# z619850002/CVIDS

Hardware: AMD Instinct MI355X
Metric: depth frames/sec integrated + Mvoxel-updates/sec, 640x480 @ 1 cm, 1/2/4/8 GPU (higher is better)
Workload: dtype f32; 1 GPU; 640x480 depth+BGR colour stream (sphere_room, 1 agent), 1 cm voxels, chunk 16^3, InverseTruncator(1), carving 0.05 m, projective TSDF integration + marching cubes every 10 frames; image=640x480, chunk=16, color=True, frames_per_call=10, mesh_every=10, parallelism=1 GPU

## Files before the change

### cvids_amd/capi.py

```python
import ctypes as C
import os
import subprocess

_HERE = os.path.dirname(os.path.abspath(__file__))
_LIB = os.path.join(_HERE, os.environ.get("CHISEL_HIP_LIB", "libchisel_hip.so"))

ABI_VERSION = 3
NUM_COUNTERS = 9
COUNTER_NAMES = ["sdf", "col", "col_sat", "probe", "carved", "work_chunks", "new_chunks", "updated_chunks", "frames"]
NUM_KERNELS = 6
KERNEL_NAMES = ["pyramid", "cull", "integrate", "mesh", "resolve", "cloud"]
TRUNC_CONSTANT, TRUNC_INVERSE, TRUNC_QUADRATIC = 0, 1, 2
STATUS = {0: "OK", 1: "ERR_INVALID", 2: "ERR_HIP", 3: "ERR_POOL_FULL", 4: "ERR_NOT_FOUND", 5: "ERR_UNSUPPORTED", 6: "ERR_IO"}


class ChiselHipError(RuntimeError):
    def __init__(self, code, msg):
        super().__init__("chisel_hip: %s (%d): %s" % (STATUS.get(code, "?"), code, msg))
        self.code = code


class Config(C.Structure):
    _fields_ = [("chunk_size", C.c_int * 3), ("voxel_resolution", C.c_float), ("use_color", C.c_int),
                ("device_id", C.c_int), ("max_chunks", C.c_int64), ("n_shards", C.c_int), ("shard_rank", C.c_int),
# ... 66 lines not shown
    "chisel_hip_meshes_to_update", "chisel_hip_meshes_to_update_since", "chisel_hip_meshes_to_update_prefetch", "chisel_hip_shell_plan_device", "chisel_hip_shell_segment_bytes", "chisel_hip_export_shells_packed", "chisel_hip_import_shells_packed", "chisel_hip_update_meshes_planned", "chisel_hip_shell_plan_queue", "chisel_hip_import_shells_fixed", "chisel_hip_shell_commit", "chisel_hip_num_meshes", "chisel_hip_list_meshes", "chisel_hip_mesh_size",
    "chisel_hip_download_mesh", "chisel_hip_get_sdf", "chisel_hip_get_sdf_and_gradient", "chisel_hip_save_ply",
    "chisel_hip_save_map", "chisel_hip_load_map",
    "chisel_hip_drop_ghost_chunks", "chisel_hip_update_meshes_of", "chisel_hip_condition_depth", "chisel_hip_condition_color", "chisel_hip_publish_cloud",
    "chisel_hip_depth_filter_create", "chisel_hip_depth_filter_destroy", "chisel_hip_depth_filter_update", "chisel_hip_depth_filter_read",
    "chisel_hip_stereo_default_params", "chisel_hip_stereo_create", "chisel_hip_stereo_destroy", "chisel_hip_stereo_set_reference",
    "chisel_hip_stereo_update", "chisel_hip_stereo_output", "chisel_hip_stereo_clear", "chisel_hip_stereo_read",
    "chisel_hip_stereo_set_camera", "chisel_hip_stereo_set_reference_image", "chisel_hip_stereo_update_image",
    "chisel_hip_stereo_bind_sparse_points", "chisel_hip_stereo_output_image", "chisel_hip_stereo_homography",
    "chisel_hip_get_counters", "chisel_hip_memory_statistics", "chisel_hip_topology_epoch", "chisel_hip_candidates", "chisel_hip_cloud_candidates", "chisel_hip_mesh_cube", "chisel_hip_write_mesh_ply", "chisel_hip_shade_vertices", "chisel_hip_generate_mesh", "chisel_hip_recompute_mesh", "chisel_hip_integrate_chunk", "chisel_hip_dirty_ids_device", "chisel_hip_mesh_shell_plan",
    "chisel_hip_shell_volume", "chisel_hip_set_profiling", "chisel_hip_get_profile", "chisel_hip_get_launch_stats", "chisel_hip_pool_info", "chisel_hip_mc_tables", "chisel_hip_mesh_cube_values", "chisel_hip_interpolate_vertex", "chisel_hip_raycast", "chisel_hip_chunk_owner", "chisel_hip_frustum", "chisel_hip_frustum_from_vectors", "chisel_hip_create_group", "chisel_hip_render_view",
    "chisel_hip_query_points", "chisel_hip_cast_rays", "chisel_hip_align_terms", "chisel_hip_align_solve", "chisel_hip_align_depth",
]
SELFTEST_EXPORTS = [
    "chisel_hip_kat_truncation", "chisel_hip_kat_dist", "chisel_hip_kat_color", "chisel_hip_kat_color_fresh", "chisel_hip_kat_color_any",
    "chisel_hip_kat_reciprocal", "chisel_hip_kat_floor", "chisel_hip_kat_raycast", "chisel_hip_debug_cloud_stats",
    "chisel_hip_debug_cull_space", "chisel_hip_debug_frustum_range", "chisel_hip_debug_stereo_prep",
]


def library_path():
    return _LIB


def build_library(force=False):
    src_dir = os.path.join(_HERE, "csrc")
    if not force and os.path.exists(_LIB):
        newest = max(os.path.getmtime(os.path.join(src_dir, f)) for f in os.listdir(src_dir))
        newest = max(newest, os.path.getmtime(os.path.join(_HERE, "..", "include", "chisel_hip.h")))
        if os.path.getmtime(_LIB) >= newest:
            return _LIB
# ... 115 lines not shown
    L.chisel_hip_kat_truncation.argtypes = [C.c_int, C.c_float, f32p, C.c_int, f32p, f32p]
    L.chisel_hip_kat_dist.argtypes = [f32p, C.c_int, f32p]
    L.chisel_hip_kat_color.argtypes = [u8p, C.c_int, u8p]
    for name, types in (("chisel_hip_wait_event", [vp, vp]), ("chisel_hip_record_event", [vp, vp]),
                        ("chisel_hip_order_stream_after_map", [vp, vp]), ("chisel_hip_order_map_after_stream", [vp, vp]),
                        ("chisel_hip_query_points", [vp, vp, C.c_int64, vp, vp, vp, vp, vp, C.c_int]),
                        ("chisel_hip_cast_rays", [vp, vp, C.c_int64, C.c_float, vp, vp, vp, vp, C.c_int]),
                        ("chisel_hip_align_terms", [vp, C.POINTER(DepthFrame), C.c_float, vp, C.c_int]),
                        ("chisel_hip_align_solve", [C.POINTER(C.c_double), C.c_double, C.POINTER(C.c_double)]),
                        ("chisel_hip_align_depth", [vp, C.POINTER(DepthFrame), C.POINTER(AlignParams), C.POINTER(AlignResult)]),
                        ("chisel_hip_kat_color_fresh", [C.POINTER(C.c_uint)]),
                        ("chisel_hip_kat_color_any", [C.POINTER(C.c_uint)]),
                        ("chisel_hip_debug_cloud_stats", [vp, i64p]),
                        ("chisel_hip_kat_raycast", [f32p, C.c_int, i32p, i32p, i32p, C.c_int, i32p]),
                        ("chisel_hip_kat_reciprocal", [C.POINTER(C.c_ulonglong), C.POINTER(C.c_uint)]),
                        ("chisel_hip_kat_floor", [C.POINTER(C.c_ulonglong), C.POINTER(C.c_uint)])):
        try:
            getattr(L, name).argtypes = types
        except AttributeError:
            pass
    L.chisel_hip_frustum.argtypes = [f32p, C.c_float, C.c_float, C.c_int, C.c_int, C.c_float, C.c_float, f32p, f32p, f32p]
    L.chisel_hip_debug_frustum_range.argtypes = [f32p, C.c_float, C.c_float, C.c_float, C.c_float, C.c_int, C.c_int,
                                                 C.c_int, C.c_float, i32p, i32p, f32p, f32p]
    _lib = L
    return L


def check(rc):
    if rc != 0:
        raise ChiselHipError(rc, load_library().chisel_hip_last_error().decode(errors="replace"))
```

### cvids_amd/csrc/chisel_device.h

```cpp
#pragma once
#include <hip/hip_runtime.h>
#include <stdint.h>

namespace chisel_hip {

constexpr uint64_t KEY_EMPTY = ~0ull;
constexpr uint64_t KEY_TOMB = ~0ull - 1ull;
constexpr int ID_BIAS = 1 << 20;
constexpr int INTEGRATE_MAX_GRID = 4096;
constexpr int INTEGRATE_GRID_CAP = 1 << 19;

__host__ __device__ inline uint64_t pack_id(int x, int y, int z) {
    return (uint64_t)(uint32_t)(x + ID_BIAS) | ((uint64_t)(uint32_t)(y + ID_BIAS) << 21) |
           ((uint64_t)(uint32_t)(z + ID_BIAS) << 42);
}
__host__ __device__ inline void unpack_id(uint64_t k, int &x, int &y, int &z) {
    x = (int)(k & 0x1FFFFF) - ID_BIAS;
    y = (int)((k >> 21) & 0x1FFFFF) - ID_BIAS;
    z = (int)((k >> 42) & 0x1FFFFF) - ID_BIAS;
}
__host__ __device__ inline uint64_t chunk_hash(int x, int y, int z) {
    return ((uint64_t)(int64_t)x * 73856093ull) ^ ((uint64_t)(int64_t)y * 19349663ull) ^
           ((uint64_t)(int64_t)z * 8349279ull);
}
// ... 184 lines not shown
        double r = (double)reading;
        double v = (double)kQuadTerm * (r * r) + (double)(kLinTerm * reading) + (double)kConstTerm;
        v = v < 0 ? -v : v;
        return (float)(v * (double)param);
    }
}
__device__ inline float reciprocal_in_range(float z) {
    const float r = __builtin_amdgcn_rcpf(z);
    return __builtin_fmaf(__builtin_fmaf(-z, r, 1.0f), r, r);
}
__device__ inline int floor_to_int(float x) {
    int r;
    asm("v_cvt_flr_i32_f32 %0, %1" : "=v"(r) : "v"(x));
    return r;
}
constexpr float FASTZ_MIN = 9.094947017729282e-13f;
constexpr float FASTZ_MAX = 1099511627776.0f;
__host__ __device__ inline float constant_weight(float weight, float truncation) { return weight / (5 * truncation); }
__host__ __device__ inline void dist_integrate(float &sdf, float &w, float distUpdate, float weightUpdate) {
    float newDist = (w * sdf + weightUpdate * distUpdate) / (weightUpdate + w);
    sdf = newDist;
    w = w + weightUpdate;
}
__host__ __device__ inline uint8_t color_channel(uint8_t old, uint8_t weight, uint8_t nw, uint8_t weightUpdate) {
    const unsigned x = (unsigned)weight * (unsigned)old + (unsigned)weightUpdate * (unsigned)nw;
    const unsigned d = (unsigned)weightUpdate + (unsigned)weight;
    if (d == 0u) return 0;
    const unsigned q = x / d;
    return (uint8_t)(q > 255u ? 255u : q);
}
// ... 37 lines not shown
    return *reinterpret_cast<const unaligned_u32 *>(data + lo);
}
__device__ inline unsigned color_word(unsigned raw, unsigned shift) {
    const unsigned v = raw >> shift;
    return ((v >> 16) & 0xffu) | (v & 0xff00u) | ((v & 0xffu) << 16);
}

__device__ inline unsigned color_gather2(const uint8_t *data, unsigned idx, unsigned channels, unsigned last_word, unsigned &shift) {
    const unsigned b = __umul24(idx, channels);
    const unsigned lo = b < last_word ? b : last_word;
    shift = (b - lo) * 8u;
    return *reinterpret_cast<const unaligned_u32 *>(data + lo);
}
__device__ inline unsigned color_integrate_fresh_bgr(unsigned c, unsigned v) {
    const float wf = (float)(c >> 24);
    const float r = __builtin_amdgcn_rcpf(wf + 1.0f);
    const float hr = __builtin_fmaf(0.5f, r, -0.5f);
    const float x0 = __builtin_fmaf(wf, (float)(c & 0xffu), (float)((v >> 16) & 0xffu));
    const float x1 = __builtin_fmaf(wf, (float)((c >> 8) & 0xffu), (float)((v >> 8) & 0xffu));
    const float x2 = __builtin_fmaf(wf, (float)((c >> 16) & 0xffu), (float)(v & 0xffu));
    unsigned q = c + 0x01000000u;
    q = __builtin_amdgcn_cvt_pk_u8_f32(__builtin_fmaf(x0, r, hr), 0u, q);
    q = __builtin_amdgcn_cvt_pk_u8_f32(__builtin_fmaf(x1, r, hr), 1u, q);
    q = __builtin_amdgcn_cvt_pk_u8_f32(__builtin_fmaf(x2, r, hr), 2u, q);
    return q;
}

__host__ __device__ inline bool sdf_below_carve_threshold(float sdf) { return sdf <= 1e-5f; }

}
```

### cvids_amd/csrc/chisel_hip.hip

```cpp
#include "../../include/chisel_hip.h"
#include "../../include/chisel_hip_selftest.h"

#include <hip/hip_runtime.h>
#include <hip/hip_ext.h>
#include <dlfcn.h>

#include <algorithm>
#include <array>
#include <atomic>
#include <chrono>
#include <condition_variable>
#include <functional>
#include <mutex>
#include <thread>
#include <cmath>
#include <cstdlib>
#include <cstdio>
#include <cstring>
#include <fstream>
#include <map>
#include <string>
#include <unordered_map>
#include <set>
#include <unordered_set>
// ... 2327 lines not shown
    if (ph[15])
        fprintf(stderr, "integrate_kernel phases, us per wave: item %.2f frames %.2f deposit %.2f store+or %.2f dequeue %.2f | alive %.2f | waves %llu units/wave %.2f\n",
                ph[9] * 0.01 / ph[15], ph[10] * 0.01 / ph[15], ph[11] * 0.01 / ph[15], ph[12] * 0.01 / ph[15], ph[13] * 0.01 / ph[15],
                ph[14] * 0.01 / ph[15], (unsigned long long)ph[15], (double)out[5] * 16.0 / ph[15]);
    if (ph[15])
        fprintf(stderr, "   units %llu (%.2f per wave)  frames visited %.2f per unit, executed %.2f per unit (%.2f us each), with a band update %.2f per unit\n",
                (unsigned long long)ph[19], (double)ph[19] / ph[15], (double)ph[16] / ph[19], (double)ph[17] / ph[19], ph[17] ? ph[18] * 0.01 / ph[17] : 0.0, (double)ph[20] / ph[19]);
    if (ph[15]) {
        uint64_t u[6] = {0, 0, 0, 0, 0, 0};
        for (int b = 0; b < 64; b++)
            for (int c = 0; c < 3; c++) { u[c] += rows[(size_t)b * 16 + 13 + c]; u[3 + c] += rows[(size_t)(64 + b) * 16 + 13 + c]; }
        const double ex = (double)ph[17];
        fprintf(stderr, "   per executed wave-frame: lanes needed %.1f / 64, voxels with a record %.1f / 256, voxels in band or carve test %.1f / 256; band code run by %.2f of them with %.1f lanes, carve code by %.2f with %.1f lanes\n",
                u[0] / ex, u[1] / ex, u[2] / ex, ph[20] / ex, ph[20] ? (double)u[3] / ph[20] : 0.0, u[5] / ex, u[5] ? (double)u[4] / u[5] : 0.0);
    }
    {
        unsigned long long mp[8];
        if (hipMemcpyFromSymbol(mp, HIP_SYMBOL(g_mesh_phase), sizeof(mp)) == hipSuccess && mp[7]) {
            fprintf(stderr, "mesh_count_kernel, us per job (thread 0): lookups %.2f | corners staged %.2f | cubes classified %.2f | scan %.2f | reserve %.2f | records %.2f | jobs %llu\n",
                    mp[0] * 0.01 / mp[7], mp[1] * 0.01 / mp[7], mp[2] * 0.01 / mp[7], mp[3] * 0.01 / mp[7], mp[4] * 0.01 / mp[7], mp[5] * 0.01 / mp[7], mp[7]);
            unsigned long long z[8] = {0, 0, 0, 0, 0, 0, 0, 0};
            (void)hipMemcpyToSymbol(HIP_SYMBOL(g_mesh_phase), z, sizeof(z));
        }
        if (hipMemcpyFromSymbol(mp, HIP_SYMBOL(g_tri_phase), sizeof(mp)) == hipSuccess && mp[7]) {
            fprintf(stderr, "mesh_triangle_kernel, us per wave (lane 0): prefix + search %.2f | record, job row, position %.2f | corners, three vertices %.2f | gradient %.2f | colour %.2f | waves sampled %llu\n",
                    mp[0] * 0.01 / mp[7], mp[1] * 0.01 / mp[7], mp[2] * 0.01 / mp[7], mp[3] * 0.01 / mp[7], mp[4] * 0.01 / mp[7], mp[7]);
            unsigned long long z[8] = {0, 0, 0, 0, 0, 0, 0, 0};
            (void)hipMemcpyToSymbol(HIP_SYMBOL(g_tri_phase), z, sizeof(z));
        }
    }
// ... 300 lines not shown
```

### cvids_amd/csrc/host_selftest.h

```cpp
extern "C" {

int chisel_hip_kat_truncation(int kind, float param, const float *depths, int n, float *trunc, float *weight1) {
    DeviceBuffer<float> d_in, d_t, d_w;
    HIP_TRY(d_in.alloc(n));
    HIP_TRY(d_t.alloc(n));
    HIP_TRY(d_w.alloc(n));
    HIP_TRY(hipMemcpy(d_in.get(), depths, n * sizeof(float), hipMemcpyHostToDevice));
    hipLaunchKernelGGL(kat_truncation_kernel, dim3((n + 255) / 256), dim3(256), 0, 0, kind, param, d_in.get(), n, d_t.get(), d_w.get());
    HIP_TRY(hipMemcpy(trunc, d_t.get(), n * sizeof(float), hipMemcpyDeviceToHost));
    HIP_TRY(hipMemcpy(weight1, d_w.get(), n * sizeof(float), hipMemcpyDeviceToHost));
    return CHISEL_HIP_OK;
}
int chisel_hip_kat_dist(const float *ops, int n, float *out) {
    DeviceBuffer<float> d_in, d_out;
    HIP_TRY(d_in.alloc(n * 3));
    HIP_TRY(d_out.alloc(n * 2));
    HIP_TRY(hipMemcpy(d_in.get(), ops, n * 3 * sizeof(float), hipMemcpyHostToDevice));
    hipLaunchKernelGGL(kat_dist_kernel, dim3(1), dim3(64), 0, 0, d_in.get(), n, d_out.get());
    HIP_TRY(hipMemcpy(out, d_out.get(), n * 2 * sizeof(float), hipMemcpyDeviceToHost));
    return CHISEL_HIP_OK;
}
int chisel_hip_kat_raycast(const float *rays, int n, const int lo[3], const int hi[3], int *cells, int cap, int *count) {
    DeviceBuffer<float> d_in;
    DeviceBuffer<int> d_cells, d_count;
// ... 67 lines not shown
    HIP_TRY(hipMemcpy(example_bits, e.get(), sizeof(unsigned), hipMemcpyDeviceToHost));
    return CHISEL_HIP_OK;
}
int chisel_hip_kat_floor(unsigned long long *mismatches, unsigned *example_bits) {
    DeviceBuffer<unsigned long long> d;
    DeviceBuffer<unsigned> e;
    HIP_TRY(d.alloc(1));
    HIP_TRY(e.alloc(1));
    HIP_TRY(hipMemset(d.get(), 0, sizeof(unsigned long long)));
    HIP_TRY(hipMemset(e.get(), 0, sizeof(unsigned)));
    hipLaunchKernelGGL(kat_floor_kernel, dim3(4096), dim3(256), 0, 0, d.get(), e.get());
    HIP_TRY(hipMemcpy(mismatches, d.get(), sizeof(unsigned long long), hipMemcpyDeviceToHost));
    HIP_TRY(hipMemcpy(example_bits, e.get(), sizeof(unsigned), hipMemcpyDeviceToHost));
    return CHISEL_HIP_OK;
}
int chisel_hip_debug_cull_space(const int range_min[3], const int range_dim[3], int n_shards, int shard_rank, int shard_block, int *ids,
                                int capacity, int *count) {
    CullParams P;
    memset(&P, 0, sizeof(P));
    for (int a = 0; a < 3; a++) {
        P.range_min[a] = range_min[a];
        P.range_dim[a] = range_dim[a];
    }
    P.ip.n_shards = n_shards;
    P.ip.shard_rank = shard_rank;
    P.ip.shard_block = shard_block;
    const CullSpace space(P);
    int n = 0;
    for (int c = 0; c < space.total; c++) {
        int x, y, z;
// ... 21 lines not shown
```

### cvids_amd/csrc/kernels_integrate.h

```cpp
#pragma once
#include <type_traits>

#include "chisel_device.h"
#include "kernels_cull.h"
#include "kernels_map.h"

namespace chisel_hip {

#ifndef INTEGRATE_WAVES
#define INTEGRATE_WAVES 6
#endif
#ifndef INTEGRATE_BLOCKS_PER_CU
#define INTEGRATE_BLOCKS_PER_CU 6
#endif
#ifndef INTEGRATE_WPB
#define INTEGRATE_WPB 1
#endif
#ifndef INTEGRATE_FINE_BELOW
#define INTEGRATE_FINE_BELOW 600
#endif

#ifndef INTEGRATE_PIPE
#define INTEGRATE_PIPE 0
#endif
#ifndef OPT_INSIDE
#define OPT_INSIDE 1
#endif
#ifndef OPT_ENDZ
#define OPT_ENDZ 1
#endif
#ifndef OPT_CARVESKIP
#define OPT_CARVESKIP 1
#endif
#ifndef OPT_COLOR2
#define OPT_COLOR2 1
#endif

constexpr int QUEUE_STRIDE = 32;
constexpr int QUEUE_HEADS = 128;

template <int N, int VPL>
struct Geom {
    static_assert(VPL == 4 || VPL == 2, "voxels per lane");
    static constexpr int V = N * N * N;
    static constexpr int QX = N / VPL;
    static constexpr int QUADS = V / VPL;
    static constexpr int LAYER_QUADS = QX * N;
    static constexpr int WPC = QUADS / 64;
    static_assert(QUADS % 64 == 0, "whole waves");
    static constexpr int BX = 2 * VPL, BY = 8, BZ = 4;
    static constexpr int NBX = N / BX, NBY = N / BY, NBZ = N / BZ;
    static_assert(NBX * NBY * NBZ == WPC && NBX >= 1 && NBY >= 1 && NBZ >= 1, "bricks tile the chunk");
// ... 153 lines not shown
            units_x = n_coarse_x * G::WPC + (n_x - n_coarse_x) * GF::WPC;
        }
    }
    const int rem_chunks = mixed ? 0 : n_items - grid_waves / G::WPC;
    const IntegratorParams &ip = P.ip;
    unsigned t_sdf = 0, t_col = 0, t_colsat = 0, t_probe = 0, t_carved = 0;
    unsigned n_new = 0, n_updated = 0;
    int shard_try = 0;
#ifdef CHISEL_PHASES
    unsigned long long ph_last_start = 0, ph_max_unit = 0, ph_exec0 = 0;
    int ph_wid = 0;
    unsigned long long ph_visit = 0, ph_exec = 0, ph_exec_t = 0, ph_units = 0, ph_band = 0, ph_fr_t = 0;
    unsigned long long ph_f[5] = {0, 0, 0, 0, 0}, ph_ft = 0;
#define FSTAMP(i, dep) do { asm volatile("" ::"v"(dep)); const unsigned long long n_ = __builtin_amdgcn_s_memrealtime(); ph_f[i] += n_ - ph_ft; ph_ft = n_; } while (0)
    unsigned long long ph_need_l = 0, ph_vox = 0, ph_band_l = 0, ph_carve_w = 0, ph_carve_l = 0, ph_bandcarve_v = 0;
    unsigned long long ph[6] = {0, 0, 0, 0, 0, 0}, ph_t = __builtin_amdgcn_s_memrealtime(), ph_t0 = ph_t;
#define PHASE(i) do { const unsigned long long n_ = __builtin_amdgcn_s_memrealtime(); ph[i] += n_ - ph_t; ph_t = n_; } while (0)
#else
#define PHASE(i) do { } while (0)
#define FSTAMP(i, dep) do { } while (0)
#endif

    auto run_unit = [&](auto vpl_tag, const int it, const int wq, const int wid) {
            constexpr int VPL = decltype(vpl_tag)::value;
            using G = Geom<N, VPL>;
            using QuadF = QuadFT<VPL>;
            using QuadU = QuadUT<VPL>;
            PHASE0(1, n_items);
            const WorkItem wi = items[it];
            int cr_flags = 0;
// ... 50 lines not shown
#pragma unroll
            for (int j = 0; j < VPL; j++) {
                s4.v[j] = 99999.0f;
                w4.v[j] = 0.0f;
                c4.v[j] = 0u;
            }
            constexpr unsigned HAVE = 1u, HAVEC = 2u, DCHG = 4u, CCHG = 8u;
            unsigned st = existed ? 0u : (HAVE | HAVEC);
            const size_t slot_base = (size_t)(existed ? slot : 0) * G::V;
            const unsigned lane_off = (unsigned)((vz * N + vy) * N + vx0);
            unsigned bm = 0u, cm = 0u;
            int carve_v = 0;

            struct Proj {
                int k, flags;
                bool need;
                float pcz[VPL];
                unsigned off[VPL];
                PixelRec r[VPL];
            };
            auto project = [&](const int k) -> Proj {
                Proj pj;
                pj.k = k;
#ifdef CHISEL_PHASES
                ph_ft = __builtin_amdgcn_s_memrealtime();
                ph_fr_t = ph_ft;
                ph_visit++;
#endif
                const int flags = __builtin_amdgcn_readlane(cr_flags, k);
                pj.flags = flags;
                const FrameCam &F = P.f[k];
                const CameraParams &C = F.cam;
                const float dy = wy - C.t[1], dz = wz - C.t[2];
                const float s2 = C.R[5] * dy + C.R[8] * dz;
                float dx[VPL];
                float (&pcz)[VPL] = pj.pcz;
#pragma unroll
                for (int j = 0; j < VPL; j++) {
                    dx[j] = wx[j] - C.t[0];
                    pcz[j] = C.R[2] * dx[j] + s2;
                }
                const bool need = true;
                pj.need = need;
                FSTAMP(0, (int)need);
                if (need && !(st & HAVE)) {
                    s4 = *reinterpret_cast<const QuadF *>((M.sdf + slot_base) + lane_off);
                    w4 = *reinterpret_cast<const QuadF *>((M.wgt + slot_base) + lane_off);
                    st |= HAVE;
                }
                if (COLOR && need && !(st & HAVEC)) {
                    c4 = *reinterpret_cast<const QuadU *>((M.rgbw + slot_base) + lane_off);
                    st |= HAVEC;
                }
                unsigned (&off)[VPL] = pj.off;
                PixelRec (&r)[VPL] = pj.r;
                const float s0 = C.R[3] * dy + C.R[6] * dz;
                const float s1 = C.R[4] * dy + C.R[7] * dz;
                float inv_z[VPL];
                if (flags & WI_FASTZ) {
#pragma unroll
                    for (int j = 0; j < VPL; j++) inv_z[j] = reciprocal_in_range(pcz[j]);
                } else {
#pragma unroll
                    for (int j = 0; j < VPL; j++) inv_z[j] = 1.0f / pcz[j];
                }
                const char *rec_base = reinterpret_cast<const char *>(F.rec - 1);
                const unsigned row_bytes = (unsigned)C.W * (unsigned)sizeof(PixelRec);
                float zn[VPL];
                if (OPT_INSIDE && (flags & WI_INSIDE)) {
                    const unsigned nm = need ? 0xffffffffu : 0u;
#pragma unroll
                    for (int j = 0; j < VPL; j++) {
                        const float pcx = C.R[0] * dx[j] + s0, pcy = C.R[1] * dx[j] + s1;
                        const float u = C.fx * pcx * inv_z[j] + C.cx;
                        const float v = C.fy * pcy * inv_z[j] + C.cy;
                        const unsigned iu = (unsigned)floor_to_int(u), iv = (unsigned)floor_to_int(v);
                        off[j] = (__umul24(iv, row_bytes) + ((iu << 3) + 8u)) & nm;
                        r[j] = *reinterpret_cast<const PixelRec *>(rec_base + off[j]);
                    }
                } else {
#pragma unroll
                for (int j = 0; j < VPL; j++) zn[j] = need ? pcz[j] : -1.0f;
#pragma unroll
                for (int j = 0; j < VPL; j++) {
                    const float pcx = C.R[0] * dx[j] + s0, pcy = C.R[1] * dx[j] + s1;
                    const float u = C.fx * pcx * inv_z[j] + C.cx;
                    const float v = C.fy * pcy * inv_z[j] + C.cy;
                    const int iu = floor_to_int(u), iv = floor_to_int(v);
                    const int iv_ok = ((unsigned)iu < (unsigned)C.W) ? iv : -1;
                    const float z_ok = ((unsigned)iv_ok < (unsigned)C.H) ? zn[j] : -1.0f;
                    off[j] = (z_ok > 0.0f) ? __umul24((unsigned)iv, row_bytes) + ((unsigned)iu + 1u) * (unsigned)sizeof(PixelRec) : 0u;
#ifdef CHISEL_ABLATE_GATHER
                    r[j] = *reinterpret_cast<const PixelRec *>(rec_base + (off[j] ? (unsigned)((lane * VPL + j + 1) * sizeof(PixelRec)) : 0u));
#else
                    r[j] = *reinterpret_cast<const PixelRec *>(rec_base + off[j]);
#endif
                }
                }
                FSTAMP(1, off[VPL - 1]);
                return pj;
            };
            auto apply = [&](const Proj &pj) {
                const int k = pj.k, flags = pj.flags;
                const FrameCam &F = P.f[k];
                const float (&pcz)[VPL] = pj.pcz;
                const unsigned (&off)[VPL] = pj.off;
                const PixelRec (&r)[VPL] = pj.r;
                float sd[VPL];
                unsigned bandm = 0u, carvem = 0u;
#if OPT_CARVESKIP
#pragma unroll
                for (int j = 0; j < VPL; j++) sd[j] = r[j].x - pcz[j];
// ... 6 lines not shown
                    for (int j = 0; j < VPL; j++) carvem |= (sd[j] > r[j].y + ip.carving_dist) ? (1u << j) : 0u;
                    carvem &= ~bandm;
                }
#else
#pragma unroll
                for (int j = 0; j < VPL; j++) {
                    sd[j] = r[j].x - pcz[j];
                    bandm |= (fabsf(sd[j]) < r[j].y + ip.diag) ? (1u << j) : 0u;
                    carvem |= (sd[j] > r[j].y + ip.carving_dist) ? (1u << j) : 0u;
                }
                carvem = ip.carving ? (carvem & ~bandm) : 0u;
#endif
                FSTAMP(2, bandm | carvem);
                t_sdf += (unsigned)__popc(bandm);
#ifdef CHISEL_PHASES
                ph_need_l += __builtin_popcountll(__ballot(pj.need));
                for (int j = 0; j < VPL; j++) ph_vox += __builtin_popcountll(__ballot(off[j] != 0u));
                ph_band_l += __builtin_popcountll(__ballot(bandm != 0u));
                ph_carve_l += __builtin_popcountll(__ballot(carvem != 0u));
                for (int j = 0; j < VPL; j++) ph_bandcarve_v += __builtin_popcountll(__ballot(((bandm | carvem) >> j) & 1u));
                if (__any(carvem != 0u)) ph_carve_w++;
#endif
                if (existed) {
                    t_probe += (unsigned)__popc(carvem);
                } else {
                    unsigned frame_carve = 0u;
#pragma unroll
                    for (int j = 0; j < VPL; j++) frame_carve += wave_count((carvem >> j) & 1u);
                    carve_v = (lane == k) ? (int)frame_carve : carve_v;
                }
                if (__any(bandm != 0u)) {
#ifdef CHISEL_PHASES
                    ph_band++;
#endif
                    bm |= 1u << k;
                    cm |= 1u << k;
                    unsigned cw[VPL], csh[VPL];
                    unsigned lastm = 0u;
                    int cpix[VPL];
                    unsigned freshm = 0u;
                    const bool word_gather = COLOR && F.color_channels >= 3;
                    if (COLOR) {
                        const unsigned image_bytes = (unsigned)(F.ccam.W * F.ccam.H * F.color_channels);
                        unsigned hasm = 0u;
#pragma unroll
                        for (int j = 0; j < VPL; j++) {
                            cpix[j] = SAMECAM ? (int)(off[j] / (unsigned)sizeof(PixelRec)) - 1
                                              : (((bandm >> j) & 1u) ? color_pixel(F.ccam, wx[j], wy, wz) : -1);
                            if (!SAMECAM) hasm |= (cpix[j] >= 0) ? (1u << j) : 0u;
                            freshm |= ((u4(c4, j) >> 24) < 8u) ? (1u << j) : 0u;
                        }
                        if (SAMECAM) hasm = bandm;
                        else hasm &= bandm;
                        freshm &= hasm;
                        t_col += (unsigned)__popc(freshm);
                        if (!SAMECAM) t_colsat += (unsigned)__popc(hasm & ~freshm);
                        if (OPT_COLOR2 && word_gather && __any(freshm != 0u)) {
                            const unsigned last_word = image_bytes - 4u;
                            lastm = 0u;
#pragma unroll
                            for (int j = 0; j < VPL; j++) {
                                unsigned sh;
                                cw[j] = color_gather2(F.color, ((freshm >> j) & 1u) ? (unsigned)cpix[j] : 0u, (unsigned)F.color_channels, last_word, sh);
                                lastm |= sh ? (1u << j) : 0u;
                            }
                        } else if (word_gather && __any(freshm != 0u)) {
#pragma unroll
                            for (int j = 0; j < VPL; j++)
#ifdef CHISEL_ABLATE_GATHER
                                cw[j] = color_gather(F.color, ((freshm >> j) & 1u) ? lane * VPL + j : 0, F.color_channels, image_bytes, csh[j]);
#else
                                cw[j] = color_gather(F.color, ((freshm >> j) & 1u) ? cpix[j] : 0, F.color_channels, image_bytes, csh[j]);
#endif
                        }
                    }
                    float wu[VPL];
                    if (COLOR && (flags & WI_FASTWU)) {
#pragma unroll
                        for (int j = 0; j < VPL; j++) wu[j] = reciprocal_in_range(5.0f * r[j].y);
                    } else {
#pragma unroll
                        for (int j = 0; j < VPL; j++) wu[j] = COLOR ? constant_weight(ip.weight, r[j].y) : 1.0f;
                    }
#pragma unroll
                    for (int j = 0; j < VPL; j++) {
                        float ns = f4(s4, j), nw = f4(w4, j);
                        dist_integrate(ns, nw, sd[j], wu[j]);
                        const bool in_band = ((bandm >> j) & 1u) != 0u;
                        f4(s4, j) = in_band ? ns : f4(s4, j);
                        f4(w4, j) = in_band ? nw : f4(w4, j);
                    }
                    st |= bandm ? DCHG : 0u;
                    if (COLOR && __any(freshm != 0u)) {
                        if (word_gather) {
#pragma unroll
                            for (int j = 0; j < VPL; j++) {
                                const unsigned nc = OPT_COLOR2 ? color_integrate_fresh_bgr(u4(c4, j), cw[j] >> (((lastm >> j) & 1u) * 8u))
                                                               : color_integrate_fresh(u4(c4, j), color_word(cw[j], csh[j]));
                                u4(c4, j) = ((freshm >> j) & 1u) ? nc : u4(c4, j);
                            }
                        } else {
#pragma unroll
                            for (int j = 0; j < VPL; j++) {
                                if ((freshm >> j) & 1u) {
                                    unsigned cbits = u4(c4, j);
                                    uchar4 cv = *reinterpret_cast<uchar4 *>(&cbits);
                                    uint8_t cr, cg, cb;
                                    color_at(F.color, cpix[j], F.color_channels, cr, cg, cb);
                                    cv = color_integrate(cv, cr, cg, cb, 1);
                                    u4(c4, j) = *reinterpret_cast<unsigned *>(&cv);
                                }
                            }
// ... 18 lines not shown
                        const bool decay = COLOR && !(f4(w4, j) < 5.0f);
                        const float cw_ = decay ? f4(w4, j) - 1.0f : 0.0f;
                        const float cs_ = decay ? f4(s4, j) : 99999.0f;
                        f4(w4, j) = hit ? cw_ : f4(w4, j);
                        f4(s4, j) = hit ? cs_ : f4(s4, j);
                    }
                    t_carved += (unsigned)__popc(hitm);
                    st |= hitm ? DCHG : 0u;
                    if (__any(hitm != 0u)) cm |= 1u << k;
                }
#ifdef CHISEL_PHASES
                FSTAMP(4, f4(s4, 0));
                ph_exec++;
                ph_exec_t += __builtin_amdgcn_s_memrealtime() - ph_fr_t;
#endif
            };
#if INTEGRATE_PIPE
            if (mask) {
                Proj cur = project(__builtin_ctz(mask));
                mask &= mask - 1u;
                while (true) {
                    const bool more = mask != 0u;
                    Proj nxt = cur;
                    if (more) {
                        nxt = project(__builtin_ctz(mask));
                        mask &= mask - 1u;
                    }
                    apply(cur);
                    if (!more) break;
                    cur = nxt;
// ... 106 lines not shown
        for (int i = 0; i < 5; i++) atomicAdd(&row[9 + i], ph[i]);
        atomicAdd(&row[14], ph_t - ph_t0);
        atomicAdd(&row[15], 1ull);
        unsigned long long *row2 = M.block_counters + (size_t)INTEGRATE_MAX_GRID * 16 + (size_t)(blockIdx.x & (INTEGRATE_MAX_GRID - 1)) * 16;
        atomicMax(&row2[5], ~ph_t0); atomicMax(&row2[6], ph_t); atomicMax(&row2[7], ph_last_start); atomicMax(&row2[8], ph_max_unit);
        if (wave == 0) { row2[9] = ph_t0; row2[10] = ph_t; row2[11] = ph_units; row2[12] = ph_exec; }
        atomicAdd(&row2[0], ph_visit); atomicAdd(&row2[1], ph_exec); atomicAdd(&row2[2], ph_exec_t); atomicAdd(&row2[3], ph_units); atomicAdd(&row2[4], ph_band);
        unsigned long long *row3 = M.block_counters + (size_t)INTEGRATE_MAX_GRID * 16 + (size_t)(blockIdx.x & 63) * 16;
        atomicAdd(&row3[13], ph_need_l); atomicAdd(&row3[14], ph_vox); atomicAdd(&row3[15], ph_bandcarve_v);
        unsigned long long *row4 = M.block_counters + (size_t)INTEGRATE_MAX_GRID * 16 + (size_t)(64 + (blockIdx.x & 63)) * 16;
        atomicAdd(&row4[13], ph_band_l); atomicAdd(&row4[14], ph_carve_l); atomicAdd(&row4[15], ph_carve_w);
        unsigned long long *row5 = M.block_counters + (size_t)INTEGRATE_MAX_GRID * 16 + (size_t)(128 + (blockIdx.x & 63)) * 16;
        atomicAdd(&row5[13], ph_f[0]); atomicAdd(&row5[14], ph_f[1]); atomicAdd(&row5[15], ph_f[2]);
        unsigned long long *row6 = M.block_counters + (size_t)INTEGRATE_MAX_GRID * 16 + (size_t)(192 + (blockIdx.x & 63)) * 16;
        atomicAdd(&row6[13], ph_f[3]); atomicAdd(&row6[14], ph_f[4]);
    }
#endif
    unsigned sums[5] = {t_sdf, t_col, (COLOR && SAMECAM) ? (t_sdf - t_col) : t_colsat, t_probe, t_carved};
#pragma unroll
    for (int c = 0; c < 5; c++)
#pragma unroll
        for (int o = 32; o > 0; o >>= 1) sums[c] += __shfl_down(sums[c], o);
    if (lane == 0) {
        unsigned long long *row = M.block_counters + (size_t)(blockIdx.x & (INTEGRATE_MAX_GRID - 1)) * 16;
        const unsigned vals[8] = {sums[0], sums[1], sums[2], sums[3], sums[4], 0u, n_new, n_updated};
#pragma unroll
        for (int k = 0; k < 8; k++)
            if (vals[k]) atomicAdd(&row[k], (unsigned long long)vals[k]);
        if (blockIdx.x == 0 && wave == 0) {
            atomicAdd(&row[5], (unsigned long long)n_items);
// ... 39 lines not shown
```

### cvids_amd/csrc/kernels_map.h

```cpp
#pragma once
#include "chisel_device.h"

namespace chisel_hip {

__device__ inline void fill_default_chunk(const MapView &M, int slot, int V) {
    float4 *s4 = reinterpret_cast<float4 *>(M.sdf + (size_t)slot * V);
    float4 *w4 = reinterpret_cast<float4 *>(M.wgt + (size_t)slot * V);
    uint4 *c4 = M.rgbw ? reinterpret_cast<uint4 *>(M.rgbw + (size_t)slot * V) : nullptr;
    for (int i = threadIdx.x; i < V / 4; i += blockDim.x) {
        s4[i] = make_float4(99999.0f, 99999.0f, 99999.0f, 99999.0f);
        w4[i] = make_float4(0.0f, 0.0f, 0.0f, 0.0f);
        if (c4) c4[i] = make_uint4(0u, 0u, 0u, 0u);
    }
}

__global__ __launch_bounds__(256) void reset_map_kernel(MapView M, int V, int all_slots) {
    __shared__ int s_list[256];
    __shared__ int s_n;
    const uint64_t gid = (uint64_t)blockIdx.x * blockDim.x + threadIdx.x;
    const uint64_t stride = (uint64_t)gridDim.x * blockDim.x;
    for (uint64_t i = gid; i <= M.hash_mask; i += stride) M.hash_keys[i] = KEY_EMPTY;
    for (uint64_t i = gid; i < (uint64_t)M.committed; i += stride) {
        M.slot_dirty[i] = 0;
        slot_summary(M)[i] = 0;
// ... 866 lines not shown
__global__ void kat_floor_kernel(unsigned long long *mismatches, unsigned *example) {
    const unsigned long long stride = (unsigned long long)gridDim.x * blockDim.x;
    unsigned long long bad = 0;
    for (unsigned long long i = (unsigned long long)blockIdx.x * blockDim.x + threadIdx.x; i < (1ull << 32); i += stride) {
        const float x = __uint_as_float((unsigned)i);
        const int got = floor_to_int(x);
        const bool ok = (x == x) ? (got == (int)floorf(x)) : ((unsigned)got >= (1u << 27));
        if (!ok) {
            bad++;
            *example = (unsigned)i;
        }
    }
    if (bad) atomicAdd(mismatches, bad);
}

}
```

### include/chisel_hip_selftest.h

```cpp
#ifndef CHISEL_HIP_SELFTEST_H_
#define CHISEL_HIP_SELFTEST_H_
#include "chisel_hip.h"
#ifdef __cplusplus
extern "C" {
#endif

int chisel_hip_kat_truncation(int kind, float param, const float *depths, int n, float *trunc, float *weight1);
int chisel_hip_kat_dist(const float *ops, int n, float *out);
int chisel_hip_kat_color(const uint8_t *ops, int n, uint8_t *out);
int chisel_hip_kat_color_fresh(unsigned *mismatches);
int chisel_hip_kat_color_any(unsigned *mismatches);
int chisel_hip_kat_reciprocal(unsigned long long *mismatches, unsigned *example_bits);
int chisel_hip_kat_floor(unsigned long long *mismatches, unsigned *example_bits);
int chisel_hip_kat_raycast(const float *rays, int n, const int lo[3], const int hi[3], int *cells, int cap, int *count);
int chisel_hip_debug_cloud_stats(chisel_hip_map *map, int64_t out[4]);
int chisel_hip_debug_cull_space(const int range_min[3], const int range_dim[3], int n_shards, int shard_rank, int shard_block, int *ids,
                                int capacity, int *count);
int chisel_hip_debug_frustum_range(const float *pose, float near_plane, float far_plane, float fy, float cy, int W, int H, int chunk_n,
                                   float res, int *range_min3, int *range_dim3, float *planes24, float *corners24);
int chisel_hip_debug_stereo_prep(chisel_hip_stereo *s, int which, void *dst);

#ifdef __cplusplus
}
#endif
#endif
```

Measured before the change: 106,000 frames/s.

## Micro-optimise integrate kernel: fused offset asm, lazy colour pixel math, explicit vmcnt wait

Several instruction-level tweaks to the TSDF integrate inner loop. Pixel record offsets now come from a two-instruction inline asm (mad_u24 plus lshl_add), and the dead 'need' mask is removed. The SAMECAM colour pixel index is computed only when a fresh colour exists, and the last-word shift mask is computed only when some index could exceed the image end. A full vmcnt(0) wait is added at the end of each frame step. New self-test and phase counters are also added. The extra waitcnt could reduce memory overlap, and the asm barriers constrain the scheduler.

Result: no change. 106,500 frames/s (median of 5 runs) (+0.4%).

```diff
diff --git a/cvids_amd/capi.py b/cvids_amd/capi.py
--- a/cvids_amd/capi.py
+++ b/cvids_amd/capi.py
@@ -104,7 +104,7 @@
 ]
 SELFTEST_EXPORTS = [
     "chisel_hip_kat_truncation", "chisel_hip_kat_dist", "chisel_hip_kat_color", "chisel_hip_kat_color_fresh", "chisel_hip_kat_color_any",
-    "chisel_hip_kat_reciprocal", "chisel_hip_kat_floor", "chisel_hip_kat_raycast", "chisel_hip_debug_cloud_stats",
+    "chisel_hip_kat_reciprocal", "chisel_hip_kat_floor", "chisel_hip_kat_record_offset", "chisel_hip_kat_raycast", "chisel_hip_debug_cloud_stats",
     "chisel_hip_debug_cull_space", "chisel_hip_debug_frustum_range", "chisel_hip_debug_stereo_prep",
 ]
 
@@ -250,7 +250,8 @@
                         ("chisel_hip_debug_cloud_stats", [vp, i64p]),
                         ("chisel_hip_kat_raycast", [f32p, C.c_int, i32p, i32p, i32p, C.c_int, i32p]),
                         ("chisel_hip_kat_reciprocal", [C.POINTER(C.c_ulonglong), C.POINTER(C.c_uint)]),
-                        ("chisel_hip_kat_floor", [C.POINTER(C.c_ulonglong), C.POINTER(C.c_uint)])):
+                        ("chisel_hip_kat_floor", [C.POINTER(C.c_ulonglong), C.POINTER(C.c_uint)]),
+                        ("chisel_hip_kat_record_offset", [C.POINTER(C.c_ulonglong), C.POINTER(C.c_uint)])):
         try:
             getattr(L, name).argtypes = types
         except AttributeError:
diff --git a/cvids_amd/csrc/chisel_device.h b/cvids_amd/csrc/chisel_device.h
--- a/cvids_amd/csrc/chisel_device.h
+++ b/cvids_amd/csrc/chisel_device.h
@@ -222,6 +222,11 @@
     asm("v_cvt_flr_i32_f32 %0, %1" : "=v"(r) : "v"(x));
     return r;
 }
+__device__ inline unsigned record_offset(unsigned row, unsigned col, unsigned row_bytes) {
+    unsigned r;
+    asm("v_mad_u32_u24 %0, %1, %2, 8\n\tv_lshl_add_u32 %0, %3, 3, %0" : "=&v"(r) : "v"(row), "s"(row_bytes), "v"(col));
+    return r;
+}
 constexpr float FASTZ_MIN = 9.094947017729282e-13f;
 constexpr float FASTZ_MAX = 1099511627776.0f;
 __host__ __device__ inline float constant_weight(float weight, float truncation) { return weight / (5 * truncation); }
@@ -289,7 +294,9 @@
 }
 __device__ inline unsigned color_integrate_fresh_bgr(unsigned c, unsigned v) {
     const float wf = (float)(c >> 24);
-    const float r = __builtin_amdgcn_rcpf(wf + 1.0f);
+    float d = wf;
+    asm("" : "+v"(d));
+    const float r = __builtin_amdgcn_rcpf(d + 1.0f);
     const float hr = __builtin_fmaf(0.5f, r, -0.5f);
     const float x0 = __builtin_fmaf(wf, (float)(c & 0xffu), (float)((v >> 16) & 0xffu));
     const float x1 = __builtin_fmaf(wf, (float)((c >> 8) & 0xffu), (float)((v >> 8) & 0xffu));
diff --git a/cvids_amd/csrc/chisel_hip.hip b/cvids_amd/csrc/chisel_hip.hip
--- a/cvids_amd/csrc/chisel_hip.hip
+++ b/cvids_amd/csrc/chisel_hip.hip
@@ -2365,6 +2365,14 @@
         fprintf(stderr, "   per executed wave-frame: lanes needed %.1f / 64, voxels with a record %.1f / 256, voxels in band or carve test %.1f / 256; band code run by %.2f of them with %.1f lanes, carve code by %.2f with %.1f lanes\n",
                 u[0] / ex, u[1] / ex, u[2] / ex, ph[20] / ex, ph[20] ? (double)u[3] / ph[20] : 0.0, u[5] / ex, u[5] ? (double)u[4] / u[5] : 0.0);
     }
+    if (ph[15] && ph[17]) {
+        uint64_t s[3] = {0, 0, 0};
+        for (int b = 0; b < 64; b++)
+            for (int c = 0; c < 3; c++) s[c] += rows[(size_t)(256 + b) * 16 + 13 + c];
+        fprintf(stderr, "   executed wave-frames %llu: without WI_FASTZ %llu (%.4f), without WI_INSIDE %llu (%.4f); with a band update %llu, of them without WI_FASTWU %llu (%.4f)\n",
+                (unsigned long long)ph[17], (unsigned long long)s[0], (double)s[0] / ph[17], (unsigned long long)s[2], (double)s[2] / ph[17],
+                (unsigned long long)ph[20], (unsigned long long)s[1], ph[20] ? (double)s[1] / ph[20] : 0.0);
+    }
     {
         unsigned long long mp[8];
         if (hipMemcpyFromSymbol(mp, HIP_SYMBOL(g_mesh_phase), sizeof(mp)) == hipSuccess && mp[7]) {
diff --git a/cvids_amd/csrc/host_selftest.h b/cvids_amd/csrc/host_selftest.h
--- a/cvids_amd/csrc/host_selftest.h
+++ b/cvids_amd/csrc/host_selftest.h
@@ -105,6 +105,19 @@
     HIP_TRY(hipMemcpy(example_bits, e.get(), sizeof(unsigned), hipMemcpyDeviceToHost));
     return CHISEL_HIP_OK;
 }
+int chisel_hip_kat_record_offset(unsigned long long *mismatches, unsigned *example) {
+    DeviceBuffer<unsigned long long> d;
+    DeviceBuffer<unsigned> e;
+    HIP_TRY(d.alloc(1));
+    HIP_TRY(e.alloc(1));
+    HIP_TRY(hipMemset(d.get(), 0, sizeof(unsigned long long)));
+    HIP_TRY(hipMemset(e.get(), 0, sizeof(unsigned)));
+    for (unsigned w : {1u, 2u, 3u, 64u, 640u, 1241u, 1280u, 4095u, 4096u})
+        hipLaunchKernelGGL(kat_record_offset_kernel, dim3(1024), dim3(256), 0, 0, w * (unsigned)sizeof(PixelRec), d.get(), e.get());
+    HIP_TRY(hipMemcpy(mismatches, d.get(), sizeof(unsigned long long), hipMemcpyDeviceToHost));
+    HIP_TRY(hipMemcpy(example, e.get(), sizeof(unsigned), hipMemcpyDeviceToHost));
+    return CHISEL_HIP_OK;
+}
 int chisel_hip_debug_cull_space(const int range_min[3], const int range_dim[3], int n_shards, int shard_rank, int shard_block, int *ids,
                                 int capacity, int *count) {
     CullParams P;
diff --git a/cvids_amd/csrc/kernels_integrate.h b/cvids_amd/csrc/kernels_integrate.h
--- a/cvids_amd/csrc/kernels_integrate.h
+++ b/cvids_amd/csrc/kernels_integrate.h
@@ -35,7 +35,17 @@
 #ifndef OPT_COLOR2
 #define OPT_COLOR2 1
 #endif
-
+#ifndef OPT_NO_STALE_WAIT
+#define OPT_NO_STALE_WAIT 1
+#endif
+#ifndef OPT_OFFSET2
+#define OPT_OFFSET2 1
+#endif
+#ifndef OPT_COLOR3
+#define OPT_COLOR3 1
+#endif
+
+constexpr int WAIT_VMCNT0 = 0x0f70;
 constexpr int QUEUE_STRIDE = 32;
 constexpr int QUEUE_HEADS = 128;
 
@@ -219,6 +229,7 @@
     unsigned long long ph_f[5] = {0, 0, 0, 0, 0}, ph_ft = 0;
 #define FSTAMP(i, dep) do { asm volatile("" ::"v"(dep)); const unsigned long long n_ = __builtin_amdgcn_s_memrealtime(); ph_f[i] += n_ - ph_ft; ph_ft = n_; } while (0)
     unsigned long long ph_need_l = 0, ph_vox = 0, ph_band_l = 0, ph_carve_w = 0, ph_carve_l = 0, ph_bandcarve_v = 0;
+    unsigned long long ph_slow_z = 0, ph_slow_wu = 0, ph_outside = 0;
     unsigned long long ph[6] = {0, 0, 0, 0, 0, 0}, ph_t = __builtin_amdgcn_s_memrealtime(), ph_t0 = ph_t;
 #define PHASE(i) do { const unsigned long long n_ = __builtin_amdgcn_s_memrealtime(); ph[i] += n_ - ph_t; ph_t = n_; } while (0)
 #else
@@ -299,7 +310,6 @@
 
             struct Proj {
                 int k, flags;
-                bool need;
                 float pcz[VPL];
                 unsigned off[VPL];
                 PixelRec r[VPL];
@@ -325,20 +335,17 @@
                     dx[j] = wx[j] - C.t[0];
                     pcz[j] = C.R[2] * dx[j] + s2;
                 }
-                const bool need = true;
-                pj.need = need;
-                FSTAMP(0, (int)need);
-                if (need && !(st & HAVE)) {
+                FSTAMP(0, pcz[0]);
+                if (!(st & HAVE)) {
                     s4 = *reinterpret_cast<const QuadF *>((M.sdf + slot_base) + lane_off);
                     w4 = *reinterpret_cast<const QuadF *>((M.wgt + slot_base) + lane_off);
                     st |= HAVE;
                 }
-                if (COLOR && need && !(st & HAVEC)) {
+                if (COLOR && !(st & HAVEC)) {
                     c4 = *reinterpret_cast<const QuadU *>((M.rgbw + slot_base) + lane_off);
                     st |= HAVEC;
                 }
                 unsigned (&off)[VPL] = pj.off;
-                PixelRec (&r)[VPL] = pj.r;
                 const float s0 = C.R[3] * dy + C.R[6] * dz;
                 const float s1 = C.R[4] * dy + C.R[7] * dz;
                 float inv_z[VPL];
@@ -351,36 +358,35 @@
                 }
                 const char *rec_base = reinterpret_cast<const char *>(F.rec - 1);
                 const unsigned row_bytes = (unsigned)C.W * (unsigned)sizeof(PixelRec);
-                float zn[VPL];
                 if (OPT_INSIDE && (flags & WI_INSIDE)) {
-                    const unsigned nm = need ? 0xffffffffu : 0u;
 #pragma unroll
                     for (int j = 0; j < VPL; j++) {
                         const float pcx = C.R[0] * dx[j] + s0, pcy = C.R[1] * dx[j] + s1;
                         const float u = C.fx * pcx * inv_z[j] + C.cx;
                         const float v = C.fy * pcy * inv_z[j] + C.cy;
                         const unsigned iu = (unsigned)floor_to_int(u), iv = (unsigned)floor_to_int(v);
-                        off[j] = (__umul24(iv, row_bytes) + ((iu << 3) + 8u)) & nm;
-                        r[j] = *reinterpret_cast<const PixelRec *>(rec_base + off[j]);
+                        off[j] = OPT_OFFSET2 ? record_offset(iv, iu, row_bytes) : __umul24(iv, row_bytes) + ((iu << 3) + 8u);
                     }
                 } else {
 #pragma unroll
-                for (int j = 0; j < VPL; j++) zn[j] = need ? pcz[j] : -1.0f;
+                    for (int j = 0; j < VPL; j++) {
+                        const float pcx = C.R[0] * dx[j] + s0, pcy = C.R[1] * dx[j] + s1;
+                        const float u = C.fx * pcx * inv_z[j] + C.cx;
+                        const float v = C.fy * pcy * inv_z[j] + C.cy;
+                        const int iu = floor_to_int(u), iv = floor_to_int(v);
+                        const int iv_ok = ((unsigned)iu < (unsigned)C.W) ? iv : -1;
+                        const float z_ok = ((unsigned)iv_ok < (unsigned)C.H) ? pcz[j] : -1.0f;
+                        off[j] = !(z_ok > 0.0f) ? 0u : OPT_OFFSET2 ? record_offset((unsigned)iv, (unsigned)iu, row_bytes) : __umul24((unsigned)iv, row_bytes) + ((unsigned)iu + 1u) * (unsigned)sizeof(PixelRec);
+                    }
+                }
+                PixelRec (&r)[VPL] = pj.r;
 #pragma unroll
                 for (int j = 0; j < VPL; j++) {
-                    const float pcx = C.R[0] * dx[j] + s0, pcy = C.R[1] * dx[j] + s1;
-                    const float u = C.fx * pcx * inv_z[j] + C.cx;
-                    const float v = C.fy * pcy * inv_z[j] + C.cy;
-                    const int iu = floor_to_int(u), iv = floor_to_int(v);
-                    const int iv_ok = ((unsigned)iu < (unsigned)C.W) ? iv : -1;
-                    const float z_ok = ((unsigned)iv_ok < (unsigned)C.H) ? zn[j] : -1.0f;
-                    off[j] = (z_ok > 0.0f) ? __umul24((unsigned)iv, row_bytes) + ((unsigned)iu + 1u) * (unsigned)sizeof(PixelRec) : 0u;
 #ifdef CHISEL_ABLATE_GATHER
                     r[j] = *reinterpret_cast<const PixelRec *>(rec_base + (off[j] ? (unsigned)((lane * VPL + j + 1) * sizeof(PixelRec)) : 0u));
 #else
                     r[j] = *reinterpret_cast<const PixelRec *>(rec_base + off[j]);
 #endif
-                }
                 }
                 FSTAMP(1, off[VPL - 1]);
                 return pj;
@@ -417,12 +423,15 @@
                 FSTAMP(2, bandm | carvem);
                 t_sdf += (unsigned)__popc(bandm);
 #ifdef CHISEL_PHASES
-                ph_need_l += __builtin_popcountll(__ballot(pj.need));
+                ph_need_l += __builtin_popcountll(__ballot(true));
                 for (int j = 0; j < VPL; j++) ph_vox += __builtin_popcountll(__ballot(off[j] != 0u));
                 ph_band_l += __builtin_popcountll(__ballot(bandm != 0u));
                 ph_carve_l += __builtin_popcountll(__ballot(carvem != 0u));
                 for (int j = 0; j < VPL; j++) ph_bandcarve_v += __builtin_popcountll(__ballot(((bandm | carvem) >> j) & 1u));
                 if (__any(carvem != 0u)) ph_carve_w++;
+                if (!(flags & WI_FASTZ)) ph_slow_z++;
+                if (!(flags & WI_INSIDE)) ph_outside++;
+                if (COLOR && !(flags & WI_FASTWU) && __any(bandm != 0u)) ph_slow_wu++;
 #endif
                 if (existed) {
                     t_probe += (unsigned)__popc(carvem);
@@ -443,14 +452,16 @@
                     int cpix[VPL];
                     unsigned freshm = 0u;
                     const bool word_gather = COLOR && F.color_channels >= 3;
+                    bool any_fresh = false;
                     if (COLOR) {
                         const unsigned image_bytes = (unsigned)(F.ccam.W * F.ccam.H * F.color_channels);
                         unsigned hasm = 0u;
 #pragma unroll
                         for (int j = 0; j < VPL; j++) {
-                            cpix[j] = SAMECAM ? (int)(off[j] / (unsigned)sizeof(PixelRec)) - 1
-                                              : (((bandm >> j) & 1u) ? color_pixel(F.ccam, wx[j], wy, wz) : -1);
-                            if (!SAMECAM) hasm |= (cpix[j] >= 0) ? (1u << j) : 0u;
+                            if (!SAMECAM) {
+                                cpix[j] = ((bandm >> j) & 1u) ? color_pixel(F.ccam, wx[j], wy, wz) : -1;
+                                hasm |= (cpix[j] >= 0) ? (1u << j) : 0u;
+                            }
                             freshm |= ((u4(c4, j) >> 24) < 8u) ? (1u << j) : 0u;
                         }
                         if (SAMECAM) hasm = bandm;
@@ -458,16 +469,35 @@
                         freshm &= hasm;
                         t_col += (unsigned)__popc(freshm);
                         if (!SAMECAM) t_colsat += (unsigned)__popc(hasm & ~freshm);
-                        if (OPT_COLOR2 && word_gather && __any(freshm != 0u)) {
+                        any_fresh = __any(freshm != 0u);
+                        if (SAMECAM && (any_fresh || !OPT_COLOR3)) {
+#pragma unroll
+                            for (int j = 0; j < VPL; j++) {
+                                unsigned o = off[j];
+                                if (OPT_COLOR3) asm volatile("" : "+v"(o));
+                                cpix[j] = (int)(o / (unsigned)sizeof(PixelRec)) - 1;
+                            }
+                        }
+                        if (OPT_COLOR2 && word_gather && any_fresh) {
                             const unsigned last_word = image_bytes - 4u;
                             lastm = 0u;
+                            unsigned bmax = 0u;
 #pragma unroll
                             for (int j = 0; j < VPL; j++) {
                                 unsigned sh;
-                                cw[j] = color_gather2(F.color, ((freshm >> j) & 1u) ? (unsigned)cpix[j] : 0u, (unsigned)F.color_channels, last_word, sh);
-                                lastm |= sh ? (1u << j) : 0u;
+                                const unsigned idx = ((freshm >> j) & 1u) ? (unsigned)cpix[j] : 0u;
+                                cw[j] = color_gather2(F.color, idx, (unsigned)F.color_channels, last_word, sh);
+                                const unsigned b = __umul24(idx, (unsigned)F.color_channels);
+                                bmax = b > bmax ? b : bmax;
                             }
-                        } else if (word_gather && __any(freshm != 0u)) {
+                            if (!OPT_COLOR3 || __any(bmax > last_word)) {
+#pragma unroll
+                                for (int j = 0; j < VPL; j++) {
+                                    const unsigned idx = ((freshm >> j) & 1u) ? (unsigned)cpix[j] : 0u;
+                                    lastm |= (__umul24(idx, (unsigned)F.color_channels) > last_word) ? (1u << j) : 0u;
+                                }
+                            }
+                        } else if (word_gather && any_fresh) {
 #pragma unroll
                             for (int j = 0; j < VPL; j++)
 #ifdef CHISEL_ABLATE_GATHER
@@ -494,11 +524,15 @@
                         f4(w4, j) = in_band ? nw : f4(w4, j);
                     }
                     st |= bandm ? DCHG : 0u;
-                    if (COLOR && __any(freshm != 0u)) {
+                    if (COLOR && any_fresh) {
                         if (word_gather) {
+                            if (OPT_COLOR2 && (!OPT_COLOR3 || __any(lastm != 0u))) {
+#pragma unroll
+                                for (int j = 0; j < VPL; j++) cw[j] >>= ((lastm >> j) & 1u) * 8u;
+                            }
 #pragma unroll
                             for (int j = 0; j < VPL; j++) {
-                                const unsigned nc = OPT_COLOR2 ? color_integrate_fresh_bgr(u4(c4, j), cw[j] >> (((lastm >> j) & 1u) * 8u))
+                                const unsigned nc = OPT_COLOR2 ? color_integrate_fresh_bgr(u4(c4, j), cw[j])
                                                                : color_integrate_fresh(u4(c4, j), color_word(cw[j], csh[j]));
                                 u4(c4, j) = ((freshm >> j) & 1u) ? nc : u4(c4, j);
                             }
@@ -547,6 +581,7 @@
                 ph_exec++;
                 ph_exec_t += __builtin_amdgcn_s_memrealtime() - ph_fr_t;
 #endif
+                if (OPT_NO_STALE_WAIT) __builtin_amdgcn_s_waitcnt(WAIT_VMCNT0);
             };
 #if INTEGRATE_PIPE
             if (mask) {
@@ -683,6 +718,8 @@
         atomicAdd(&row5[13], ph_f[0]); atomicAdd(&row5[14], ph_f[1]); atomicAdd(&row5[15], ph_f[2]);
         unsigned long long *row6 = M.block_counters + (size_t)INTEGRATE_MAX_GRID * 16 + (size_t)(192 + (blockIdx.x & 63)) * 16;
         atomicAdd(&row6[13], ph_f[3]); atomicAdd(&row6[14], ph_f[4]);
+        unsigned long long *row7 = M.block_counters + (size_t)INTEGRATE_MAX_GRID * 16 + (size_t)(256 + (blockIdx.x & 63)) * 16;
+        atomicAdd(&row7[13], ph_slow_z); atomicAdd(&row7[14], ph_slow_wu); atomicAdd(&row7[15], ph_outside);
     }
 #endif
     unsigned sums[5] = {t_sdf, t_col, (COLOR && SAMECAM) ? (t_sdf - t_col) : t_colsat, t_probe, t_carved};
diff --git a/cvids_amd/csrc/kernels_map.h b/cvids_amd/csrc/kernels_map.h
--- a/cvids_amd/csrc/kernels_map.h
+++ b/cvids_amd/csrc/kernels_map.h
@@ -904,4 +904,18 @@
     if (bad) atomicAdd(mismatches, bad);
 }
 
-}
+__global__ void kat_record_offset_kernel(unsigned row_bytes, unsigned long long *mismatches, unsigned *example) {
+    const unsigned stride = gridDim.x * blockDim.x;
+    unsigned long long bad = 0;
+    for (unsigned i = blockIdx.x * blockDim.x + threadIdx.x; i < (1u << 24); i += stride) {
+        const unsigned row = i >> 12, col = i & 4095u;
+        const unsigned want = __umul24(row, row_bytes) + ((col << 3) + 8u);
+        if (record_offset(row, col, row_bytes) != want) {
+            bad++;
+            *example = (row << 16) | col;
+        }
+    }
+    if (bad) atomicAdd(mismatches, bad);
+}
+
+}
diff --git a/include/chisel_hip_selftest.h b/include/chisel_hip_selftest.h
--- a/include/chisel_hip_selftest.h
+++ b/include/chisel_hip_selftest.h
@@ -12,6 +12,7 @@
 int chisel_hip_kat_color_any(unsigned *mismatches);
 int chisel_hip_kat_reciprocal(unsigned long long *mismatches, unsigned *example_bits);
 int chisel_hip_kat_floor(unsigned long long *mismatches, unsigned *example_bits);
+int chisel_hip_kat_record_offset(unsigned long long *mismatches, unsigned *example);
 int chisel_hip_kat_raycast(const float *rays, int n, const int lo[3], const int hi[3], int *cells, int cap, int *count);
 int chisel_hip_debug_cloud_stats(chisel_hip_map *map, int64_t out[4]);
 int chisel_hip_debug_cull_space(const int range_min[3], const int range_dim[3], int n_shards, int shard_rank, int shard_block, int *ids,
```
